# w-k-jones/tobac-flow

Hardware: AMD Instinct MI355X
Metric: Mpix/s end-to-end flow+sobel+watershed, 5424^2 frames (higher is better)
Workload: dtype f32

## Files before the change

tobac_flow_amd/csrc/watershed.hip:

```cpp
#include "tf_common.h"
#include <string.h>
#include <time.h>
#include <stdio.h>
#include <stdlib.h>
#include "tf_prim.h"
#include <new>

typedef unsigned long long u64;
#define WS_INF 0xFFFFFFFFFFFFFFFFull
#define WS_MARKER_BIT 0x8000000000000000ull
#define WS_MAX_NBR 26
#define WS_MAX_DEPTH TF_WS_MAX_DEPTH
#define WS_BATCH 32
#define WS_K2(c, i) ((c).KM[2 * (int64_t)(i)])
#define WS_M1(c, i) ((c).KM[2 * (int64_t)(i) + 1])

struct WsGeom {
    int64_t T; int H, W; int64_t plane;
    int n_nbr;
    int8_t dt[WS_MAX_NBR], dy[WS_MAX_NBR], dx[WS_MAX_NBR];
    int n_tx;
};

#ifndef WS_TILE
#define WS_TILE 16
#endif
__device__ __forceinline__ int64_t ws_vpos(const WsGeom &g, int64_t t, int y, int x) {
    const int64_t tile = (int64_t)(y / WS_TILE) * g.n_tx + x / WS_TILE;
    return ((tile * g.T + t) * WS_TILE + (y % WS_TILE)) * WS_TILE + (x % WS_TILE);
}
static int64_t ws_virtual_voxels(int64_t T, int64_t H, int64_t W) {
    return T * ((H + WS_TILE - 1) / WS_TILE * WS_TILE) * ((W + WS_TILE - 1) / WS_TILE * WS_TILE);
}

struct WsC {
    int64_t R; int n_nbr;
    const u64 *pix; const unsigned *val; const int *nbr;
    u64 *KM;
    u64 *C[WS_MAX_DEPTH], *Rt;
    int *Llo, *Lhi;
    const u64 *emask;
};

__device__ __forceinline__ unsigned ws_ordkey(float v) {
    v = v + 0.0f;
    unsigned u = __float_as_uint(v);
    return (u & 0x80000000u) ? ~u : (u | 0x80000000u);
}
__device__ __forceinline__ u64 ws_load(const u64 *p) {
    return __hip_atomic_load(p, __ATOMIC_RELAXED, __HIP_MEMORY_SCOPE_AGENT);
}
__device__ __forceinline__ int ws_round_flow(float f) {
    return (f == f) ? __float2int_rn(f) : 0;
}

__device__ __forceinline__ int64_t ws_neighbour(const WsGeom &g, int64_t t, int y, int x, int fx, int fy, int bx, int by, int i) {
    const int dt = g.dt[i];
    int yy = y + g.dy[i], xx = x + g.dx[i];
    if (dt == 1) { xx += fx; yy += fy; }
    else if (dt == -1) { xx += bx; yy += by; }
    const int64_t tt = t + dt;
    if (tt < 0 || tt >= g.T || (unsigned)yy >= (unsigned)g.H || (unsigned)xx >= (unsigned)g.W) return -1;
    return tt * g.plane + (int64_t)yy * g.W + xx;
}

__global__ void __launch_bounds__(256)
k_ws_classify(const int32_t *__restrict__ markers, const int8_t *__restrict__ mask, int64_t n, uint8_t *__restrict__ cls)
{
    const int64_t i = (int64_t)blockIdx.x * blockDim.x + threadIdx.x;
    if (i >= n) return;
    const int32_t m = markers[i];
// ... 144 lines not shown
    for (int j = 0; j < 4; j++) { f[j] = ((w >> (8 * j)) & 0xffu) != 0; m[j] = __ballot(f[j]); before += __popcll(m[j] & below); }
    if (y >= g.H || x0 >= g.W) return;
    const int64_t p0 = t * g.plane + (int64_t)y * g.W + x0;
    const int id0 = (int)base[b] + before;
    int c[4], run = 0;
#pragma unroll
    for (int j = 0; j < 4; j++) {
        c[j] = -1;
        if (f[j]) { const int id = id0 + run; c[j] = cls[p0 + j] == 1 ? id : -2 - id; run++; }
    }
    if (x0 + 3 < g.W && (((uintptr_t)(cid + p0)) & 15) == 0) *(int4 *)(cid + p0) = make_int4(c[0], c[1], c[2], c[3]);
    else {
#pragma unroll
        for (int j = 0; j < 4; j++) if (x0 + j < g.W) cid[p0 + j] = c[j];
    }
}
static_assert(WS_TILE * WS_TILE == 256, "one scan block = one tile of one frame");

__global__ void __launch_bounds__(256)
k_ws_cid(const uint8_t *__restrict__ cls, const uint8_t *__restrict__ flag, const int *__restrict__ scan, int64_t n,
         int *__restrict__ cid)
{
    const int64_t i = (int64_t)blockIdx.x * blockDim.x + threadIdx.x;
    if (i >= n) return;
    int c = -1;
    if (flag[i]) c = cls[i] == 1 ? scan[i] : -2 - scan[i];
    cid[i] = c;
}

template <int NN>
__global__ void __launch_bounds__(256)
k_ws_compact(const float *__restrict__ field, const float *__restrict__ fwd, const float *__restrict__ bwd,
             const int *__restrict__ cid, WsGeom g, u64 *__restrict__ pix, unsigned *__restrict__ val,
             int *__restrict__ nbr, u64 *__restrict__ KM, int *__restrict__ nan_flag)
{
    const int x = blockIdx.x * 64 + threadIdx.x, y = blockIdx.y * 4 + threadIdx.y;
    const int64_t t = blockIdx.z;
    if (x >= g.W || y >= g.H) return;
    const int64_t p = t * g.plane + (int64_t)y * g.W + x;
    const int c = cid[p];
    if (c == -1) return;
    const bool marker = c < 0;
    const int64_t id = marker ? -2 - c : c;
    const float2 fw = ((const float2 *)fwd)[p], bw = ((const float2 *)bwd)[p];
    const int fx = ws_round_flow(fw.x), fy = ws_round_flow(fw.y), bx = ws_round_flow(bw.x), by = ws_round_flow(bw.y);
    const float fv = field[p];
    if (fv != fv) *nan_flag = 1;
    const unsigned v = ws_ordkey(fv);
    pix[id] = (u64)p | (marker ? WS_MARKER_BIT : 0ull);
    val[id] = v;
    if (NN > 0) {
        int cn[NN > 0 ? NN : 1];
#pragma unroll
        for (int i = 0; i < NN; i++) {
            const int64_t n = ws_neighbour(g, t, y, x, fx, fy, bx, by, i);
            const int cv = cid[n >= 0 ? n : p];
            cn[i] = n >= 0 ? cv : -1;
        }
#pragma unroll
        for (int i = 0; i < NN; i++) nbr[id * NN + i] = cn[i] < 0 ? -1 : cn[i];
    } else {
        for (int i = 0; i < g.n_nbr; i++) {
            const int64_t n = ws_neighbour(g, t, y, x, fx, fy, bx, by, i);
            int cn = -1;
            if (n >= 0) { cn = cid[n]; if (cn < 0) cn = -1; }
            nbr[id * g.n_nbr + i] = cn;
        }
    }
    *(ulonglong2 *)&KM[2 * id] = make_ulonglong2(marker ? ((u64)v << 32) : WS_INF, WS_INF);
}

struct WsRavel {
    int64_t n; int n_nbr;
    int64_t structure[WS_MAX_NBR]; int32_t floc[WS_MAX_NBR], bloc[WS_MAX_NBR];
    const int32_t *foff, *boff;
};
__device__ __forceinline__ int64_t wsr_neighbour(const WsRavel &g, int64_t p, int fo, int bo, int i) {
    const int64_t n = p + g.structure[i] + (int64_t)g.floc[i] * fo + (int64_t)g.bloc[i] * bo;
    return (n >= 0 && n < g.n) ? n : -1;
}

__global__ void __launch_bounds__(256)
k_wsr_seeds(const int64_t *__restrict__ locs, int64_t n_locs, int64_t n, uint8_t *__restrict__ seed, int *__restrict__ bad)
{
    const int64_t i = (int64_t)blockIdx.x * blockDim.x + threadIdx.x;
    if (i >= n_locs) return;
    const int64_t p = locs[i];
    if (p < 0 || p >= n || (i > 0 && locs[i - 1] >= p)) { *bad = 1; return; }
    seed[p] = 1;
}

__global__ void __launch_bounds__(256)
k_wsr_classify(const uint8_t *__restrict__ seed, const int32_t *__restrict__ output, const int8_t *__restrict__ mask, int64_t n,
               uint8_t *__restrict__ cls, int *__restrict__ bad)
{
    const int64_t i = (int64_t)blockIdx.x * blockDim.x + threadIdx.x;
    if (i >= n) return;
    const bool sd = seed[i] != 0;
    if (sd && output[i] == 0) *bad = 2;
    cls[i] = sd ? 2 : ((mask[i] != 0 && output[i] == 0) ? 1 : 0);
}

__global__ void __launch_bounds__(256)
k_wsr_relevant(const uint8_t *__restrict__ cls, WsRavel g, uint8_t *__restrict__ flag)
{
    const int64_t p = (int64_t)blockIdx.x * blockDim.x + threadIdx.x;
    if (p >= g.n) return;
    const uint8_t c = cls[p];
    uint8_t f = c == 1;
    if (c == 2) {
        const int fo = g.foff[p], bo = g.boff[p];
        for (int i = 0; i < g.n_nbr && !f; i++) { const int64_t n = wsr_neighbour(g, p, fo, bo, i); f |= n >= 0 && cls[n] == 1; }
    }
    flag[p] = f;
}

__global__ void __launch_bounds__(256)
k_wsr_compact(const float *__restrict__ image, const int *__restrict__ cid, WsRavel g, u64 *__restrict__ pix,
              unsigned *__restrict__ val, int *__restrict__ nbr, u64 *__restrict__ KM, int *__restrict__ nan_flag)
{
    const int64_t p = (int64_t)blockIdx.x * blockDim.x + threadIdx.x;
    if (p >= g.n) return;
    const int c = cid[p];
    if (c == -1) return;
    const bool marker = c < 0;
    const int64_t id = marker ? -2 - c : c;
    const int fo = g.foff[p], bo = g.boff[p];
    const float fv = image[p];
    if (fv != fv) *nan_flag = 1;
    const unsigned v = ws_ordkey(fv);
    pix[id] = (u64)p | (marker ? WS_MARKER_BIT : 0ull);
    val[id] = v;
    for (int i = 0; i < g.n_nbr; i++) {
        const int64_t n = wsr_neighbour(g, p, fo, bo, i);
        int cn = -1;
        if (n >= 0) { cn = cid[n]; if (cn < 0) cn = -1; }
        nbr[id * g.n_nbr + i] = cn;
    }
    *(ulonglong2 *)&KM[2 * id] = make_ulonglong2(marker ? ((u64)v << 32) : WS_INF, WS_INF);
}

__global__ void __launch_bounds__(256)
k_wsr_labels(const int *__restrict__ cid, const u64 *__restrict__ Rt, const u64 *__restrict__ pix, int ranked, int32_t *output, int64_t n)
{
    const int64_t i = (int64_t)blockIdx.x * blockDim.x + threadIdx.x;
    if (i >= n) return;
    const int c = cid[i];
    if (c >= 0 && output[i] == 0) { const u64 r = Rt[c]; if (r != WS_INF) output[i] = output[ranked ? (pix[r & 0xFFFFFFFFull] & ~WS_MARKER_BIT) : r]; }
}

__global__ void __launch_bounds__(256)
k_ws_init_level(const u64 *__restrict__ pix, u64 *__restrict__ dst, int64_t R, int is_root, const int *__restrict__ rank)
{
    const int64_t i = (int64_t)blockIdx.x * blockDim.x + threadIdx.x;
    if (i >= R) return;
    const u64 px = pix[i];
    const bool marker = (px & WS_MARKER_BIT) != 0ull;
    const u64 root = rank ? (((u64)(unsigned)rank[i] << 32) | (u64)(unsigned)i) : (px & ~WS_MARKER_BIT);
    dst[i] = marker ? (is_root ? root : 0ull) : WS_INF;
}

__global__ void __launch_bounds__(256)
k_ws_init_labelset(const u64 *__restrict__ pix, const int32_t *__restrict__ markers, int *__restrict__ lo,
                   int *__restrict__ hi, int64_t R)
{
    const int64_t i = (int64_t)blockIdx.x * blockDim.x + threadIdx.x;
    if (i >= R) return;
    const u64 px = pix[i];
    const bool marker = (px & WS_MARKER_BIT) != 0ull;
    const int32_t l = marker ? markers[px & ~WS_MARKER_BIT] : 0;
    lo[i] = marker ? l : 0x7fffffff;
    hi[i] = marker ? l : (int)0x80000000;
}

#define WS_LOCAL_ROUNDS 4
#ifndef WS_LDS_CAP
#define WS_LDS_CAP 4096
#endif
struct WsStage { int cnt[2]; int base; int buf[2][WS_LDS_CAP]; };

__device__ __forceinline__ void ws_stage(WsStage &st, int w, bool enq, int n, int *__restrict__ qout, int *__restrict__ cnt_out, int qcap) {
    if (enq) {
        const int pos = atomicAdd(&st.cnt[w], 1);
        if (pos < WS_LDS_CAP) st.buf[w][pos] = n;
        else { const int g = atomicAdd(cnt_out, 1); if (g < qcap) qout[g] = n; }
    }
}
__device__ __forceinline__ void ws_flush(WsStage &st, int w, int *__restrict__ qout, int *__restrict__ cnt_out, int qcap) {
    __syncthreads();
    const int n = min(st.cnt[w], WS_LDS_CAP);
    if (n > 0) {
        if (threadIdx.x == 0) st.base = atomicAdd(cnt_out, n);
        __syncthreads();
        const int base = st.base;
        for (int i = threadIdx.x; i < n; i += blockDim.x) { const int pos = base + i; if (pos < qcap) qout[pos] = st.buf[w][i]; }
        __syncthreads();
        if (threadIdx.x == 0) st.cnt[w] = 0;
    }
    __syncthreads();
}

template <class Entry>
__device__ __forceinline__ void ws_sweep(int64_t R, const int *__restrict__ qin, const int *__restrict__ cnt_in,
                                         int *__restrict__ qout, int *__restrict__ cnt_out, int qcap, Entry entry)
{
    __shared__ WsStage st;
    if (threadIdx.x == 0) { st.cnt[0] = 0; st.cnt[1] = 0; }
    __syncthreads();
    const int64_t n_in = qin ? (int64_t)min(*cnt_in, qcap) : R;
    const int64_t n_pad = (n_in + 255) & ~255ll;
    for (int64_t i0 = (int64_t)blockIdx.x * 256; i0 < n_pad; i0 += (int64_t)gridDim.x * 256) {
        const int64_t i = i0 + threadIdx.x;
        const bool act = i < n_in;
        int w = 0;
        entry(st, w, act, act ? (qin ? qin[i] : (int)i) : 0);
        for (int r = 0; r < WS_LOCAL_ROUNDS; r++) {
            __syncthreads();
            const int n = min(st.cnt[w], WS_LDS_CAP);
            if (n == 0) break;
            for (int j0 = 0; j0 < n; j0 += 256) {
                const int j = j0 + threadIdx.x;
                const bool a2 = j < n;
                entry(st, w ^ 1, a2, a2 ? st.buf[w][j] : 0);
            }
            __syncthreads();
            if (threadIdx.x == 0) st.cnt[w] = 0;
            w ^= 1;
        }
        ws_flush(st, w, qout, cnt_out, qcap);
    }
}

#define WS_NB 8

template <int NN>
__device__ __forceinline__ void ws_entry_a(const WsC &c, WsStage &st, int w, bool act, int p,
                                           int *__restrict__ qout, int *__restrict__ cnt_out, int qcap)
{
    constexpr int NB = NN ? NN : WS_NB;
    const int n_nbr = NN ? NN : c.n_nbr;
    const int *np = c.nbr + (int64_t)p * n_nbr;
    u64 kp = WS_INF;
    for (int s0 = 0; s0 < n_nbr; s0 += NB) {
        int n[NB];
#pragma unroll
        for (int j = 0; j < NB; j++) n[j] = (act && s0 + j < n_nbr) ? np[s0 + j] : -1;
        if (s0 == 0 && act) kp = ws_load(&WS_K2(c, p));
        const u64 lp = kp >> 32;
        u64 vn[NB], m1[NB], k2[NB];
#pragma unroll
        for (int j = 0; j < NB; j++) {
            const int q = n[j] >= 0 ? n[j] : 0;
            vn[j] = c.val[q];
            const ulonglong2 km = *(const ulonglong2 *)&WS_K2(c, q);
            k2[j] = km.x; m1[j] = km.y;
        }
        u64 cand[NB], old[NB];
#pragma unroll
        for (int j = 0; j < NB; j++) {
            cand[j] = vn[j] > lp ? ((vn[j] << 32) | 1ull) : (vn[j] == lp ? kp + 1ull : kp);
            old[j] = 0ull;
            if (n[j] >= 0) {
                if (kp < m1[j]) atomicMin(&WS_M1(c, n[j]), kp);
                if (cand[j] < k2[j]) old[j] = atomicMin(&WS_K2(c, n[j]), cand[j]);
            }
        }
#pragma unroll
        for (int j = 0; j < NB; j++)
            ws_stage(st, w, n[j] >= 0 && cand[j] < old[j], n[j], qout, cnt_out, qcap);
    }
}

template <int NN>
__global__ void __launch_bounds__(256)
k_ws_sweep_a(WsC c, const int *__restrict__ qin, const int *__restrict__ cnt_in, int *__restrict__ qout,
             int *__restrict__ cnt_out, int qcap)
{
    ws_sweep(c.R, qin, cnt_in, qout, cnt_out, qcap,
             [&](WsStage &st, int w, bool act, int p) { ws_entry_a<NN>(c, st, w, act, p, qout, cnt_out, qcap); });
}

__global__ void __launch_bounds__(256)
k_ws_edge_masks(WsC c, u64 *__restrict__ emask)
{
    const int64_t p = (int64_t)blockIdx.x * blockDim.x + threadIdx.x;
    if (p >= c.R) return;
    const u64 kp = WS_K2(c, p);
    u64 m = 0ull;
    if (kp != WS_INF) {
        const int *np = c.nbr + p * c.n_nbr;
        for (int i0 = 0; i0 < c.n_nbr; i0 += WS_NB) {
            int n[WS_NB]; u64 m1[WS_NB], kn[WS_NB]; unsigned vn[WS_NB];
#pragma unroll
            for (int j = 0; j < WS_NB; j++) n[j] = i0 + j < c.n_nbr ? np[i0 + j] : -1;
#pragma unroll
            for (int j = 0; j < WS_NB; j++) {
                const int q = n[j] >= 0 ? n[j] : 0;
                const ulonglong2 km = *(const ulonglong2 *)&WS_K2(c, q);
                kn[j] = km.x; m1[j] = km.y; vn[j] = c.val[q];
            }
#pragma unroll
            for (int j = 0; j < WS_NB; j++)
                if (n[j] >= 0 && m1[j] == kp) {
                    m |= 1ull << (i0 + j);
                    if ((kn[j] >> 32) == (u64)vn[j] && (kn[j] & 0xFFFFFFFFull) == 1ull) m |= 1ull << (32 + i0 + j);
                }
        }
    }
    emask[p] = m;
}

__device__ __forceinline__ int ws_load_i(const int *p) {
    return __hip_atomic_load(p, __ATOMIC_RELAXED, __HIP_MEMORY_SCOPE_AGENT);
}

template <int NN>
__device__ __forceinline__ void ws_entry_chain(const WsC &c, int k, int depth, u64 *__restrict__ dst, WsStage &st, int w,
                                               bool act0, int p,
                                               int *__restrict__ qout, int *__restrict__ cnt_out, int qcap)
{
    constexpr int NB = NN ? NN : WS_NB;
    const int n_nbr = NN ? NN : c.n_nbr;
    const int *np = c.nbr + (int64_t)p * n_nbr;
    const bool root = k == depth;
    u64 kp = WS_INF, own = WS_INF, em = 0ull;
    int own_lo = 0x7fffffff, own_hi = (int)0x80000000;
    u64 cp[WS_MAX_DEPTH];
    for (int s0 = 0; s0 < n_nbr; s0 += NB) {
        if (s0 == 0 && act0) {
            em = c.emask[p];
            kp = WS_K2(c, p);
            own = ws_load(&dst[p]);
            if (root) { own_lo = ws_load_i(&c.Llo[p]); own_hi = ws_load_i(&c.Lhi[p]); }
            for (int j = 1; j < k; j++) cp[j] = c.C[j][p];
        }
        int n[NB];
#pragma unroll
        for (int j = 0; j < NB; j++) n[j] = (s0 + j < n_nbr && ((em >> (s0 + j)) & 1ull)) ? np[s0 + j] : -1;
        u64 dn[NB];
        int lon[NB], hin[NB];
#pragma unroll
        for (int j = 0; j < NB; j++) {
            dn[j] = WS_INF; lon[j] = 0; hin[j] = 0;
            if (n[j] >= 0) { dn[j] = dst[n[j]]; if (root) { lon[j] = c.Llo[n[j]]; hin[j] = c.Lhi[n[j]]; } }
        }
        u64 offered[NB], old[NB];
        int olo[NB], ohi[NB];
#pragma unroll
        for (int j = 0; j < NB; j++) {
            offered[j] = WS_INF; old[j] = 0ull; olo[j] = (int)0x80000000; ohi[j] = 0x7fffffff;
            if (n[j] >= 0) {
                const bool entry = ((em >> (32 + s0 + j)) & 1ull) != 0ull;
                bool match = true;
                for (int l = 1; l < k && match; l++) {
                    const u64 offered_l = entry ? (l == 1 ? kp : cp[l - 1]) : cp[l];
                    match = offered_l == c.C[l][n[j]];
                }
                if (match) {
                    if (root) offered[j] = own;
                    else offered[j] = entry ? (k == 1 ? kp : cp[k - 1]) : own;
                    if (offered[j] != WS_INF && offered[j] < dn[j]) old[j] = atomicMin(&dst[n[j]], offered[j]);
                    if (root) {
                        if (own_lo < lon[j]) olo[j] = atomicMin(&c.Llo[n[j]], own_lo);
                        if (own_hi > hin[j]) ohi[j] = atomicMax(&c.Lhi[n[j]], own_hi);
                    }
                }
            }
        }
#pragma unroll
        for (int j = 0; j < NB; j++) {
            const bool improved = offered[j] < old[j] || (root && (own_lo < olo[j] || own_hi > ohi[j]));
            ws_stage(st, w, improved, n[j], qout, cnt_out, qcap);
        }
    }
}

template <int NN>
__global__ void __launch_bounds__(256)
k_ws_sweep_chain(WsC c, int k, int depth, const int *__restrict__ qin, const int *__restrict__ cnt_in,
                 int *__restrict__ qout, int *__restrict__ cnt_out, int qcap)
{
    u64 *dst = k == depth ? c.Rt : c.C[k];
    ws_sweep(c.R, qin, cnt_in, qout, cnt_out, qcap,
             [&](WsStage &st, int w, bool act, int p) { ws_entry_chain<NN>(c, k, depth, dst, st, w, act, p, qout, cnt_out, qcap); });
}

__global__ void __launch_bounds__(256)
k_ws_origins(WsC c, int depth, int *__restrict__ org)
{
    const int64_t p = (int64_t)blockIdx.x * blockDim.x + threadIdx.x;
    if (p >= c.R) return;
    const u64 kp = WS_K2(c, p);
    if (kp == WS_INF || c.Rt[p] == WS_INF) return;
    const int lo = c.Llo[p], hi = c.Lhi[p];
    u64 cp[WS_MAX_DEPTH];
    for (int j = 1; j < depth; j++) cp[j] = c.C[j][p];
    const u64 em = c.emask[p];
    for (int i = 0; i < c.n_nbr; i++) {
        if (!((em >> i) & 1ull)) continue;
        const int n = c.nbr[p * c.n_nbr + i];
        const bool entry = ((em >> (32 + i)) & 1ull) != 0ull;
        bool match = true;
        for (int l = 1; l < depth && match; l++) {
            const u64 offered_l = entry ? (l == 1 ? kp : cp[l - 1]) : cp[l];
            match = offered_l == c.C[l][n];
        }
        if (!match) continue;
        if (c.Llo[n] != lo || c.Lhi[n] != hi) {
            const bool complete = depth >= 2 && (c.C[depth - 1][n] & 0xFFFFFFFFull) == 0ull;
            atomicOr(&org[n], complete ? 1 : 2);
        }
    }
}

__global__ void __launch_bounds__(256)
k_ws_count_ambiguous(WsC c, const int *__restrict__ org, unsigned long long *__restrict__ cnt)
{
// ... 315 lines not shown
        TF_CHECK_HIP(tf_exclusive_sum_from(tmp, tb, it, scan + off, (int)carry, (size_t)n, s));
        int last_scan = 0; uint8_t last_flag = 0;
        TF_CHECK_HIP(hipMemcpyAsync(&last_scan, scan + off + n - 1, sizeof(int), hipMemcpyDeviceToHost, s));
        TF_CHECK_HIP(hipMemcpyAsync(&last_flag, flag + off + n - 1, 1, hipMemcpyDeviceToHost, s));
        TF_CHECK_HIP(hipStreamSynchronize(s));
        carry = (int64_t)last_scan + last_flag;
        TF_REQUIRE(carry <= 0x3fffff00ll, "tf_watershed: more than 2^30 relevant pixels in one call (use time windows)");
    }
    *total = carry;
    return TF_OK;
}

static size_t ws_full_bytes(int64_t N, int64_t NV) {
    return tf_align_up((size_t)N, 256) + tf_align_up((size_t)NV, 256) + tf_align_up((size_t)N * 4, 256) + tf_align_up((size_t)NV * 4, 256)
         + tf_align_up(ws_scan_temp_bytes(NV), 256) + tf_align_up((size_t)((N + 255) / 256) * 24 + 64, 256) + 4096;
}
static size_t ws_compact_bytes(int64_t R, int n_nbr, int depth) {
    return tf_align_up((size_t)R * 8, 256) + tf_align_up((size_t)R * 4, 256) + tf_align_up((size_t)R * 4 * n_nbr, 256)
         + (size_t)(depth + 2) * tf_align_up((size_t)R * 8, 256)
         + 2 * tf_align_up((size_t)R * 8 + 256, 256)
         + 5 * tf_align_up((size_t)R * 4, 256) + tf_align_up((size_t)R * 8, 256) + 4096;
}

extern "C" size_t tf_watershed_workspace_bytes(int64_t T, int64_t H, int64_t W, int n_nbr, int chain_depth, int64_t max_relevant)
{
    if (T <= 0 || H <= 0 || W <= 0 || chain_depth < 1 || chain_depth > WS_MAX_DEPTH || n_nbr < 1 || n_nbr > WS_MAX_NBR) return 0;
    const int64_t N = T * H * W;
    if (max_relevant <= 0 || max_relevant > N) max_relevant = N;
    return ws_full_bytes(N, ws_virtual_voxels(T, H, W)) + ws_compact_bytes(max_relevant, n_nbr, chain_depth);
}

struct WsQueues { int *q[2]; int *cnt; int qcap; int *h_cnt; int64_t *processed; };

static int ws_run_phase(const WsC &c, int phase_k, int depth, const WsQueues &Q, hipStream_t s, int64_t max_sweeps,
                        int64_t *sweeps_out, double alg_bytes = 0.0)
{
    const unsigned nbR = (unsigned)((c.R + 255) / 256);
    const unsigned nb = nbR < 2048u ? nbR : 2048u;
    TF_CHECK_HIP(hipMemsetAsync(Q.cnt, 0, (WS_BATCH + 1) * sizeof(int), s));
    int64_t sweeps = 0;
    int parity = 0;
    bool first = true;
    unsigned grid_hint = nb;
    for (;;) {
        const bool scan_batch = first;
        {
            TfProfScope ps(TFK_WS_RELAX, alg_bytes, s);
            alg_bytes = 0.0;
            for (int b = 0; b < WS_BATCH; b++) {
                const int *qin = first ? nullptr : Q.q[parity];
                const unsigned blocks = first ? nbR : grid_hint;
                if (phase_k == 0) {
                    if (c.n_nbr == 6) hipLaunchKernelGGL(k_ws_sweep_a<6>, dim3(blocks), dim3(256), 0, s, c, qin, Q.cnt + b, Q.q[parity ^ 1], Q.cnt + b + 1, Q.qcap);
                    else hipLaunchKernelGGL(k_ws_sweep_a<0>, dim3(blocks), dim3(256), 0, s, c, qin, Q.cnt + b, Q.q[parity ^ 1], Q.cnt + b + 1, Q.qcap);
                } else {
                    if (c.n_nbr == 6) hipLaunchKernelGGL(k_ws_sweep_chain<6>, dim3(blocks), dim3(256), 0, s, c, phase_k, depth, qin, Q.cnt + b, Q.q[parity ^ 1], Q.cnt + b + 1, Q.qcap);
                    else hipLaunchKernelGGL(k_ws_sweep_chain<0>, dim3(blocks), dim3(256), 0, s, c, phase_k, depth, qin, Q.cnt + b, Q.q[parity ^ 1], Q.cnt + b + 1, Q.qcap);
                }
                parity ^= 1;
                first = false;
            }
        }
        TF_CHECK_LAUNCH();
        TF_CHECK_HIP(hipMemcpyAsync(Q.h_cnt, Q.cnt, (WS_BATCH + 1) * sizeof(int), hipMemcpyDeviceToHost, s));
        TF_CHECK_HIP(hipStreamSynchronize(s));
        bool done = false, overflow = false;
        for (int b = (scan_batch ? 1 : 0); b <= WS_BATCH; b++) overflow = overflow || Q.h_cnt[b] > Q.qcap;
        for (int b = (scan_batch ? 1 : 0); b <= WS_BATCH && !overflow; b++) {
            if (Q.h_cnt[b] == 0) { done = true; break; }
            if (b < WS_BATCH) *Q.processed += Q.h_cnt[b];
        }
        sweeps += WS_BATCH;
        {
            const int64_t last = Q.h_cnt[WS_BATCH];
            int64_t gb = (last * 4 + 255) / 256;
            if (gb < 64) gb = 64;
            if (gb > (int64_t)nb) gb = nb;
            grid_hint = (unsigned)gb;
        }
        if (done) break;
        if (sweeps > max_sweeps) { tf_set_error("tf_watershed: phase %d did not converge in %lld sweeps", phase_k, (long long)sweeps); return TF_ENOCONV; }
        if (overflow) {
            first = true;
            TF_CHECK_HIP(hipMemsetAsync(Q.cnt, 0, (WS_BATCH + 1) * sizeof(int), s));
            continue;
        }
        TF_CHECK_HIP(hipMemcpyAsync(Q.cnt, Q.cnt + WS_BATCH, sizeof(int), hipMemcpyDeviceToDevice, s));
        TF_CHECK_HIP(hipMemsetAsync(Q.cnt + 1, 0, WS_BATCH * sizeof(int), s));
    }
    *sweeps_out = sweeps;
// ... 328 lines not shown
    hipStream_t s = j->s;
    const WsC &c = j->c;
    const int64_t R = j->R;
    const unsigned nbr_blocks = (unsigned)((R + 255) / 256);
    hipLaunchKernelGGL(k_ws_init_level, dim3(nbr_blocks), dim3(256), 0, s, c.pix, c.Rt, R, 1, ranked ? (const int *)j->rank_dev : (const int *)nullptr);
    hipLaunchKernelGGL(k_ws_init_labelset, dim3(nbr_blocks), dim3(256), 0, s, c.pix, j->markers, c.Llo, c.Lhi, R);
    TF_CHECK_LAUNCH();
    int64_t sw = 0;
    const int rc = ws_run_phase(c, j->depth, j->depth, j->Q, s, j->max_sweeps, &sw);
    if (rc) return rc;
    if (j->speculate_fast && j->depth == 1) j->st[1] = sw; else j->st[2 + (j->depth < 3 ? j->depth - 1 : 2)] += sw;
    j->st[12] += 1;
    TF_CHECK_HIP(hipMemsetAsync(j->org, 0, (size_t)R * sizeof(int), s));
    TF_CHECK_HIP(hipMemsetAsync(j->d_cnt, 0, 4 * sizeof(unsigned long long), s));
    hipLaunchKernelGGL(k_ws_origins, dim3(nbr_blocks), dim3(256), 0, s, c, j->depth, j->org);
    hipLaunchKernelGGL(k_ws_count_ambiguous, dim3(nbr_blocks), dim3(256), 0, s, c, j->org, j->d_cnt);
    TF_CHECK_LAUNCH();
    TF_CHECK_HIP(hipMemcpyAsync(j->h_amb, j->d_cnt, 4 * sizeof(unsigned long long), hipMemcpyDeviceToHost, s));
    TF_CHECK_HIP(hipStreamSynchronize(s));
    return TF_OK;
}

static int ws_job_sweeps(tf_ws_job *j)
{
    if (!j->sweeps_pending) return TF_OK;
    j->sweeps_pending = false;
    int64_t *st = j->st;
    const WsC &c = j->c;
    hipStream_t s = j->s;
    const unsigned nbr_blocks = (unsigned)((j->R + 255) / 256);
    int rc = ws_run_phase(c, 0, j->depth_max, j->Q, s, j->max_sweeps, &st[0], 29.0 * (double)j->N);
    if (rc) return rc;
    {
        TfProfScope ps(TFK_WS_SETUP, 0.0, s);
        hipLaunchKernelGGL(k_ws_edge_masks, dim3(nbr_blocks), dim3(256), 0, s, c, (u64 *)c.emask);
    }
    TF_CHECK_LAUNCH();
    j->speculate_fast = !((j->flags & TF_WS_SKIP_FAST_PATH) && j->depth0 > 1);
    st[5] = j->speculate_fast ? 0 : -1;
    j->depth = j->depth0;
    j->root_pending = true;
    if (j->speculate_fast) {
        j->depth = 1;
        rc = ws_root_and_check(j, false);
        if (rc) return rc;
        st[5] = j->h_amb[2] != 0;
        if (j->h_amb[2] == 0 || j->depth_max <= 1) j->root_pending = false;
        else j->depth = j->depth0;
    }
    if (j->root_pending) {
        rc = ws_chain_levels(j);
        if (rc) return rc;
    }
    st[8] = j->depth; st[9] = (int64_t)j->h_amb[0]; st[10] = (int64_t)j->h_amb[1]; st[11] = (int64_t)j->h_amb[2];
    return TF_OK;
}

static int ws_job_begin(tf_ws_job *j, const float *field, const int32_t *markers, const int8_t *mask,
                        const float *fwd, const float *bwd, int64_t T, int64_t H, int64_t W,
                        const int8_t *nbr_host, int n_nbr, int depth0, int depth_max, int flags,
                        void *ws, size_t ws_bytes, void *stream,
                        const WsRavel *rv = nullptr, const int64_t *rv_locs = nullptr, int64_t rv_n_locs = 0, int64_t spec_key = -1)
{
    int64_t *st = j->st;
    for (int i = 0; i < TF_WS_NSTATS; i++) st[i] = 0;
    TF_REQUIRE((flags & ~(TF_WS_SKIP_FAST_PATH | TF_WS_REFERENCE_ORDER | TF_WS_DEFER_SWEEPS)) == 0, "tf_watershed: unknown flag");
// ... 74 lines not shown
            long long *t_count = (long long *)scan, *t_base = t_count + n_tiles;
            hipLaunchKernelGGL(k_ws_count_tiles, dim3((unsigned)((n_tiles + 3) / 4)), dim3(256), 0, s, (const uint8_t *)flag, n_tiles, t_count);
            size_t tb = scan_bytes;
            TF_CHECK_HIP(tf_exclusive_sum(scan_tmp, tb, (const long long *)t_count, t_base, (size_t)n_tiles, s));
            long long h_last[2] = {0, 0};
            TF_CHECK_HIP(hipMemcpyAsync(&h_last[0], t_base + n_tiles - 1, sizeof(long long), hipMemcpyDeviceToHost, s));
            TF_CHECK_HIP(hipMemcpyAsync(&h_last[1], t_count + n_tiles - 1, sizeof(long long), hipMemcpyDeviceToHost, s));
            TF_CHECK_HIP(hipStreamSynchronize(s));
            R = h_last[0] + h_last[1];
            TF_REQUIRE(R <= 0x3fffff00ll, "tf_watershed: more than 2^30 relevant pixels in one call (use time windows)");
        } else {
            const int rc_scan = ws_scan_flags(flag, scan, NV, scan_tmp, scan_bytes, s, &R);
            if (rc_scan) return rc_scan;
        }
    }
    st[6] = R;
    j->R = R;
    if (ws_bytes < ws_full_bytes(N, NV) + ws_compact_bytes(R > 0 ? R : 1, n_nbr, depth_max)) {
        tf_set_error("tf_watershed: workspace too small for %lld relevant pixels", (long long)R);
        return TF_ENOMEM;
    }
    if (rv) hipLaunchKernelGGL(k_ws_cid, dim3(nb1), dim3(256), 0, s, cls, flag, scan, N, cid);
    else if (tiles) hipLaunchKernelGGL(k_ws_cid_tiles, dim3((unsigned)((NV / 256 + 3) / 4)), dim3(256), 0, s, (const uint8_t *)cls, (const uint8_t *)flag,
                                       (const long long *)((long long *)scan + NV / 256), NV / 256, g, cid);
    else hipLaunchKernelGGL(k_ws_cid_tiled, grid, block, 0, s, (const uint8_t *)cls, (const uint8_t *)flag, (const int *)scan, g, cid);
    TF_CHECK_LAUNCH();
    WsC &c = j->c; memset(&c, 0, sizeof(c));
    c.R = R; c.n_nbr = n_nbr;
    j->org = nullptr; j->rank_dev = nullptr;
    j->depth = 0;
    if (R > 0) {
        u64 *pix = ar.take<u64>(R); unsigned *val = ar.take<unsigned>(R); int *nbr = ar.take<int>(R * n_nbr);
        c.pix = pix; c.val = val; c.nbr = nbr;
        c.KM = ar.take<u64>(2 * R);
        for (int k = 1; k < depth_max; k++) c.C[k] = ar.take<u64>(R);
        c.Rt = ar.take<u64>(R);
        c.Llo = ar.take<int>(R); c.Lhi = ar.take<int>(R); j->org = ar.take<int>(R);
        j->rank_dev = ar.take<int>(R);
        u64 *emask = ar.take<u64>(R);
        c.emask = emask;
        WsQueues &Q = j->Q;
        Q.qcap = (int)(2 * R < 0x7fffff00ll ? 2 * R : 0x7fffff00ll);
        Q.q[0] = ar.take<int>(2 * R + 64); Q.q[1] = ar.take<int>(2 * R + 64);
        j->subid = ar.take<int>(R);
        Q.cnt = d_flags; Q.h_cnt = j->h_cnt; Q.processed = &st[7];
        if (!ar.ok()) { tf_set_error("tf_watershed: workspace too small"); return TF_ENOMEM; }
        int *d_nan = d_flags + WS_BATCH + 4;
        TF_CHECK_HIP(hipMemsetAsync(d_nan, 0, sizeof(int), s));
        {
            TfProfScope ps(TFK_WS_SETUP, 0.0, s);
            if (rv) hipLaunchKernelGGL(k_wsr_compact, dim3(nb1), dim3(256), 0, s, field, (const int *)cid, *rv, pix, val, nbr, c.KM, d_nan);
            else if (n_nbr == 6) hipLaunchKernelGGL(k_ws_compact<6>, grid, block, 0, s, field, fwd, bwd, cid, g, pix, val, nbr, c.KM, d_nan);
            else if (n_nbr == 18) hipLaunchKernelGGL(k_ws_compact<18>, grid, block, 0, s, field, fwd, bwd, cid, g, pix, val, nbr, c.KM, d_nan);
            else if (n_nbr == 26) hipLaunchKernelGGL(k_ws_compact<26>, grid, block, 0, s, field, fwd, bwd, cid, g, pix, val, nbr, c.KM, d_nan);
            else hipLaunchKernelGGL(k_ws_compact<0>, grid, block, 0, s, field, fwd, bwd, cid, g, pix, val, nbr, c.KM, d_nan);
        }
        TF_CHECK_LAUNCH();
        {
            int h_nan = 0;
            TF_CHECK_HIP(hipMemcpyAsync(&h_nan, d_nan, sizeof(int), hipMemcpyDeviceToHost, s));
            TF_CHECK_HIP(hipStreamSynchronize(s));
            if (h_nan) {
                tf_set_error("tf_watershed: the field is NaN at a floodable pixel or at a seed next to one; the pop order of the "
                             "reference's heap is undefined for NaN keys (detection.get_combined_edge_field maps NaN to +inf)");
                return TF_EINVAL;
            }
        }
        const int64_t max_sweeps = rv ? 4096 + 2 * R : 4096 + 512 * (T + H + W);
        j->max_sweeps = max_sweeps;
        if ((flags & TF_WS_REFERENCE_ORDER) && spec_key >= 0) {
            j->vmax = (unsigned)spec_key;
            j->speculative = true;
            const int rc_x = ws_job_export(j);
            if (rc_x) return rc_x;
        }
        j->sweeps_pending = true;
        if (flags & TF_WS_DEFER_SWEEPS) return TF_OK;
        return ws_job_sweeps(j);
    }
    st[8] = j->depth; st[9] = (int64_t)j->h_amb[0]; st[10] = (int64_t)j->h_amb[1]; st[11] = (int64_t)j->h_amb[2];
    return TF_OK;
}

static int ws_job_replay(tf_ws_job *j)
{
    if (!j->need_replay || j->replay_done) return j->replay_rc;
    const double t0 = ws_now_ms();
    int n_ranked = 0;
// ... 318 lines not shown
```

Measured before the change: 1026.

## Split K2/M1 arrays, defer M1 relaxation, specialise chain sweeps by depth

Replaces the interleaved K2/M1 array with two separate arrays. M1 updates move out of the iterative phase-0 sweep into one pass run after convergence. The chain sweep kernels get templates on level K and on root/non-root, so loops unroll, per-thread arrays shrink, and the root-only Llo/Lhi loads are skipped elsewhere. 6-neighbour kernels are capped at 64 VGPRs and the LDS staging capacity is halved, both to raise occupancy. The risks are register spills under the VGPR cap, more staging overflow into global queues with the smaller LDS buffer, and one extra full pass for M1.

```diff
diff --git a/tobac_flow_amd/csrc/watershed.hip b/tobac_flow_amd/csrc/watershed.hip
--- a/tobac_flow_amd/csrc/watershed.hip
+++ b/tobac_flow_amd/csrc/watershed.hip
@@ -12,8 +12,8 @@
 #define WS_MAX_NBR 26
 #define WS_MAX_DEPTH TF_WS_MAX_DEPTH
 #define WS_BATCH 32
-#define WS_K2(c, i) ((c).KM[2 * (int64_t)(i)])
-#define WS_M1(c, i) ((c).KM[2 * (int64_t)(i) + 1])
+#define WS_K2(c, i) ((c).K2[(int64_t)(i)])
+#define WS_M1(c, i) ((c).M1[(int64_t)(i)])
 
 struct WsGeom {
     int64_t T; int H, W; int64_t plane;
@@ -36,7 +36,7 @@
 struct WsC {
     int64_t R; int n_nbr;
     const u64 *pix; const unsigned *val; const int *nbr;
-    u64 *KM;
+    u64 *K2, *M1;
     u64 *C[WS_MAX_DEPTH], *Rt;
     int *Llo, *Lhi;
     const u64 *emask;
@@ -247,7 +247,7 @@
 __global__ void __launch_bounds__(256)
 k_ws_compact(const float *__restrict__ field, const float *__restrict__ fwd, const float *__restrict__ bwd,
              const int *__restrict__ cid, WsGeom g, u64 *__restrict__ pix, unsigned *__restrict__ val,
-             int *__restrict__ nbr, u64 *__restrict__ KM, int *__restrict__ nan_flag)
+             int *__restrict__ nbr, u64 *__restrict__ K2, u64 *__restrict__ M1, int *__restrict__ nan_flag)
 {
     const int x = blockIdx.x * 64 + threadIdx.x, y = blockIdx.y * 4 + threadIdx.y;
     const int64_t t = blockIdx.z;
@@ -282,7 +282,8 @@
             nbr[id * g.n_nbr + i] = cn;
         }
     }
-    *(ulonglong2 *)&KM[2 * id] = make_ulonglong2(marker ? ((u64)v << 32) : WS_INF, WS_INF);
+    K2[id] = marker ? ((u64)v << 32) : WS_INF;
+    M1[id] = WS_INF;
 }
 
 struct WsRavel {
@@ -332,7 +333,7 @@
 
 __global__ void __launch_bounds__(256)
 k_wsr_compact(const float *__restrict__ image, const int *__restrict__ cid, WsRavel g, u64 *__restrict__ pix,
-              unsigned *__restrict__ val, int *__restrict__ nbr, u64 *__restrict__ KM, int *__restrict__ nan_flag)
+              unsigned *__restrict__ val, int *__restrict__ nbr, u64 *__restrict__ K2, u64 *__restrict__ M1, int *__restrict__ nan_flag)
 {
     const int64_t p = (int64_t)blockIdx.x * blockDim.x + threadIdx.x;
     if (p >= g.n) return;
@@ -352,7 +353,8 @@
         if (n >= 0) { cn = cid[n]; if (cn < 0) cn = -1; }
         nbr[id * g.n_nbr + i] = cn;
     }
-    *(ulonglong2 *)&KM[2 * id] = make_ulonglong2(marker ? ((u64)v << 32) : WS_INF, WS_INF);
+    K2[id] = marker ? ((u64)v << 32) : WS_INF;
+    M1[id] = WS_INF;
 }
 
 __global__ void __launch_bounds__(256)
@@ -390,7 +392,7 @@
 
 #define WS_LOCAL_ROUNDS 4
 #ifndef WS_LDS_CAP
-#define WS_LDS_CAP 4096
+#define WS_LDS_CAP 2048
 #endif
 struct WsStage { int cnt[2]; int base; int buf[2][WS_LDS_CAP]; };
 
@@ -448,6 +450,10 @@
 
 #define WS_NB 8
 
+__device__ __forceinline__ u64 ws_cand_a(unsigned vn, unsigned lp, u64 kp) {
+    return vn > lp ? (((u64)vn << 32) | 1ull) : (vn == lp ? kp + 1ull : kp);
+}
+
 template <int NN>
 __device__ __forceinline__ void ws_entry_a(const WsC &c, WsStage &st, int w, bool act, int p,
                                            int *__restrict__ qout, int *__restrict__ cnt_out, int qcap)
@@ -461,38 +467,65 @@
 #pragma unroll
         for (int j = 0; j < NB; j++) n[j] = (act && s0 + j < n_nbr) ? np[s0 + j] : -1;
         if (s0 == 0 && act) kp = ws_load(&WS_K2(c, p));
-        const u64 lp = kp >> 32;
-        u64 vn[NB], m1[NB], k2[NB];
+        const unsigned lp = (unsigned)(kp >> 32);
+        unsigned vn[NB];
+        u64 k2[NB];
 #pragma unroll
         for (int j = 0; j < NB; j++) {
             const int q = n[j] >= 0 ? n[j] : 0;
             vn[j] = c.val[q];
-            const ulonglong2 km = *(const ulonglong2 *)&WS_K2(c, q);
-            k2[j] = km.x; m1[j] = km.y;
-        }
-        u64 cand[NB], old[NB];
+            k2[j] = WS_K2(c, q);
+        }
 #pragma unroll
         for (int j = 0; j < NB; j++) {
-            cand[j] = vn[j] > lp ? ((vn[j] << 32) | 1ull) : (vn[j] == lp ? kp + 1ull : kp);
-            old[j] = 0ull;
-            if (n[j] >= 0) {
-                if (kp < m1[j]) atomicMin(&WS_M1(c, n[j]), kp);
-                if (cand[j] < k2[j]) old[j] = atomicMin(&WS_K2(c, n[j]), cand[j]);
-            }
+            const u64 cand = ws_cand_a(vn[j], lp, kp);
+            const bool go = n[j] >= 0 && cand < k2[j];
+            k2[j] = 0ull;
+            if (go) k2[j] = atomicMin(&WS_K2(c, n[j]), cand);
         }
 #pragma unroll
         for (int j = 0; j < NB; j++)
-            ws_stage(st, w, n[j] >= 0 && cand[j] < old[j], n[j], qout, cnt_out, qcap);
-    }
-}
-
-template <int NN>
+            ws_stage(st, w, n[j] >= 0 && ws_cand_a(vn[j], lp, kp) < k2[j], n[j], qout, cnt_out, qcap);
+    }
+}
+
 __global__ void __launch_bounds__(256)
 k_ws_sweep_a(WsC c, const int *__restrict__ qin, const int *__restrict__ cnt_in, int *__restrict__ qout,
              int *__restrict__ cnt_out, int qcap)
 {
     ws_sweep(c.R, qin, cnt_in, qout, cnt_out, qcap,
-             [&](WsStage &st, int w, bool act, int p) { ws_entry_a<NN>(c, st, w, act, p, qout, cnt_out, qcap); });
+             [&](WsStage &st, int w, bool act, int p) { ws_entry_a<0>(c, st, w, act, p, qout, cnt_out, qcap); });
+}
+__global__ void __launch_bounds__(256) __attribute__((amdgpu_num_vgpr(64)))
+k_ws_sweep_a6(WsC c, const int *__restrict__ qin, const int *__restrict__ cnt_in, int *__restrict__ qout,
+              int *__restrict__ cnt_out, int qcap)
+{
+    ws_sweep(c.R, qin, cnt_in, qout, cnt_out, qcap,
+             [&](WsStage &st, int w, bool act, int p) { ws_entry_a<6>(c, st, w, act, p, qout, cnt_out, qcap); });
+}
+
+template <int NN>
+__global__ void __launch_bounds__(256)
+k_ws_sweep_m1(WsC c)
+{
+    const int64_t p = (int64_t)blockIdx.x * blockDim.x + threadIdx.x;
+    if (p >= c.R) return;
+    const u64 kp = WS_K2(c, p);
+    if (kp == WS_INF) return;
+    constexpr int NB = NN ? NN : WS_NB;
+    const int n_nbr = NN ? NN : c.n_nbr;
+    const int *np = c.nbr + p * n_nbr;
+    for (int s0 = 0; s0 < n_nbr; s0 += NB) {
+        int n[NB];
+        u64 m1[NB];
+#pragma unroll
+        for (int j = 0; j < NB; j++) n[j] = s0 + j < n_nbr ? np[s0 + j] : -1;
+#pragma unroll
+        for (int j = 0; j < NB; j++) m1[j] = WS_M1(c, n[j] >= 0 ? n[j] : 0);
+#pragma unroll
+        for (int j = 0; j < NB; j++)
+            if (n[j] >= 0 && kp < m1[j]) atomicMin(&WS_M1(c, n[j]), kp);
+    }
 }
 
 __global__ void __launch_bounds__(256)
@@ -511,8 +544,7 @@
 #pragma unroll
             for (int j = 0; j < WS_NB; j++) {
                 const int q = n[j] >= 0 ? n[j] : 0;
-                const ulonglong2 km = *(const ulonglong2 *)&WS_K2(c, q);
-                kn[j] = km.x; m1[j] = km.y; vn[j] = c.val[q];
+                kn[j] = WS_K2(c, q); m1[j] = WS_M1(c, q); vn[j] = c.val[q];
             }
 #pragma unroll
             for (int j = 0; j < WS_NB; j++)
@@ -529,75 +561,103 @@
     return __hip_atomic_load(p, __ATOMIC_RELAXED, __HIP_MEMORY_SCOPE_AGENT);
 }
 
-template <int NN>
-__device__ __forceinline__ void ws_entry_chain(const WsC &c, int k, int depth, u64 *__restrict__ dst, WsStage &st, int w,
+template <int NN, int K, bool ROOT>
+__device__ __forceinline__ void ws_entry_chain(const WsC &c, int k_rt, u64 *__restrict__ dst, const u64 *__restrict__ below, WsStage &st, int w,
                                                bool act0, int p,
                                                int *__restrict__ qout, int *__restrict__ cnt_out, int qcap)
 {
     constexpr int NB = NN ? NN : WS_NB;
     const int n_nbr = NN ? NN : c.n_nbr;
+    const int k = K ? K : k_rt;
     const int *np = c.nbr + (int64_t)p * n_nbr;
-    const bool root = k == depth;
     u64 kp = WS_INF, own = WS_INF, em = 0ull;
     int own_lo = 0x7fffffff, own_hi = (int)0x80000000;
-    u64 cp[WS_MAX_DEPTH];
+    u64 cp[K ? K : 1];
+    u64 ek = WS_INF;
+    auto offer = [&](int i, int l) -> u64 {
+        const bool entry = ((em >> (32 + i)) & 1ull) != 0ull;
+        if constexpr (K != 0) return entry ? (l == 1 ? kp : cp[l - 1]) : cp[l];
+        else return entry ? (l == 1 ? kp : c.C[l - 1][p]) : c.C[l][p];
+    };
+    auto offer_k = [&](int i) -> u64 {
+        const bool entry = ((em >> (32 + i)) & 1ull) != 0ull;
+        return (ROOT || !entry) ? own : ek;
+    };
     for (int s0 = 0; s0 < n_nbr; s0 += NB) {
         if (s0 == 0 && act0) {
             em = c.emask[p];
             kp = WS_K2(c, p);
             own = ws_load(&dst[p]);
-            if (root) { own_lo = ws_load_i(&c.Llo[p]); own_hi = ws_load_i(&c.Lhi[p]); }
-            for (int j = 1; j < k; j++) cp[j] = c.C[j][p];
+            if constexpr (ROOT) { own_lo = ws_load_i(&c.Llo[p]); own_hi = ws_load_i(&c.Lhi[p]); }
+            if constexpr (K != 0) {
+#pragma unroll
+                for (int j = 1; j < K; j++) cp[j] = c.C[j][p];
+            }
+            if constexpr (!ROOT) {
+                if constexpr (K == 1) ek = kp;
+                else if constexpr (K != 0) ek = cp[K - 1];
+                else ek = k == 1 ? kp : below[p];
+            }
         }
         int n[NB];
 #pragma unroll
         for (int j = 0; j < NB; j++) n[j] = (s0 + j < n_nbr && ((em >> (s0 + j)) & 1ull)) ? np[s0 + j] : -1;
         u64 dn[NB];
-        int lon[NB], hin[NB];
+        int lon[ROOT ? NB : 1], hin[ROOT ? NB : 1];
 #pragma unroll
         for (int j = 0; j < NB; j++) {
-            dn[j] = WS_INF; lon[j] = 0; hin[j] = 0;
-            if (n[j] >= 0) { dn[j] = dst[n[j]]; if (root) { lon[j] = c.Llo[n[j]]; hin[j] = c.Lhi[n[j]]; } }
-        }
-        u64 offered[NB], old[NB];
-        int olo[NB], ohi[NB];
+            dn[j] = WS_INF;
+            if constexpr (ROOT) { lon[j] = 0; hin[j] = 0; }
+            if (n[j] >= 0) { dn[j] = dst[n[j]]; if constexpr (ROOT) { lon[j] = c.Llo[n[j]]; hin[j] = c.Lhi[n[j]]; } }
+        }
 #pragma unroll
         for (int j = 0; j < NB; j++) {
-            offered[j] = WS_INF; old[j] = 0ull; olo[j] = (int)0x80000000; ohi[j] = 0x7fffffff;
+            const u64 seen = dn[j];
+            dn[j] = 0ull;
+            int seen_lo = 0, seen_hi = 0;
+            if constexpr (ROOT) { seen_lo = lon[j]; seen_hi = hin[j]; lon[j] = (int)0x80000000; hin[j] = 0x7fffffff; }
             if (n[j] >= 0) {
-                const bool entry = ((em >> (32 + s0 + j)) & 1ull) != 0ull;
                 bool match = true;
-                for (int l = 1; l < k && match; l++) {
-                    const u64 offered_l = entry ? (l == 1 ? kp : cp[l - 1]) : cp[l];
-                    match = offered_l == c.C[l][n[j]];
+                if constexpr (K != 0) {
+#pragma unroll
+                    for (int l = 1; l < K; l++) if (match) match = offer(s0 + j, l) == c.C[l][n[j]];
+                } else {
+                    for (int l = 1; l < k && match; l++) match = offer(s0 + j, l) == c.C[l][n[j]];
                 }
                 if (match) {
-                    if (root) offered[j] = own;
-                    else offered[j] = entry ? (k == 1 ? kp : cp[k - 1]) : own;
-                    if (offered[j] != WS_INF && offered[j] < dn[j]) old[j] = atomicMin(&dst[n[j]], offered[j]);
-                    if (root) {
-                        if (own_lo < lon[j]) olo[j] = atomicMin(&c.Llo[n[j]], own_lo);
-                        if (own_hi > hin[j]) ohi[j] = atomicMax(&c.Lhi[n[j]], own_hi);
+                    const u64 offered = offer_k(s0 + j);
+                    if (offered != WS_INF && offered < seen) dn[j] = atomicMin(&dst[n[j]], offered);
+                    if constexpr (ROOT) {
+                        if (own_lo < seen_lo) lon[j] = atomicMin(&c.Llo[n[j]], own_lo);
+                        if (own_hi > seen_hi) hin[j] = atomicMax(&c.Lhi[n[j]], own_hi);
                     }
                 }
             }
         }
 #pragma unroll
         for (int j = 0; j < NB; j++) {
-            const bool improved = offered[j] < old[j] || (root && (own_lo < olo[j] || own_hi > ohi[j]));
+            bool improved = offer_k(s0 + j) < dn[j];
+            if constexpr (ROOT) improved = improved || own_lo < lon[j] || own_hi > hin[j];
             ws_stage(st, w, improved, n[j], qout, cnt_out, qcap);
         }
     }
 }
 
-template <int NN>
-__global__ void __launch_bounds__(256)
-k_ws_sweep_chain(WsC c, int k, int depth, const int *__restrict__ qin, const int *__restrict__ cnt_in,
+template <bool ROOT>
+__global__ void __launch_bounds__(256)
+k_ws_sweep_chain(WsC c, int k, u64 *__restrict__ dst, const u64 *__restrict__ below, const int *__restrict__ qin, const int *__restrict__ cnt_in,
                  int *__restrict__ qout, int *__restrict__ cnt_out, int qcap)
 {
-    u64 *dst = k == depth ? c.Rt : c.C[k];
     ws_sweep(c.R, qin, cnt_in, qout, cnt_out, qcap,
-             [&](WsStage &st, int w, bool act, int p) { ws_entry_chain<NN>(c, k, depth, dst, st, w, act, p, qout, cnt_out, qcap); });
+             [&](WsStage &st, int w, bool act, int p) { ws_entry_chain<0, 0, ROOT>(c, k, dst, below, st, w, act, p, qout, cnt_out, qcap); });
+}
+template <int K, bool ROOT>
+__global__ void __launch_bounds__(256) __attribute__((amdgpu_num_vgpr(64)))
+k_ws_sweep_chain6(WsC c, int k, u64 *__restrict__ dst, const u64 *__restrict__ below, const int *__restrict__ qin, const int *__restrict__ cnt_in,
+                  int *__restrict__ qout, int *__restrict__ cnt_out, int qcap)
+{
+    ws_sweep(c.R, qin, cnt_in, qout, cnt_out, qcap,
+             [&](WsStage &st, int w, bool act, int p) { ws_entry_chain<6, K, ROOT>(c, k, dst, below, st, w, act, p, qout, cnt_out, qcap); });
 }
 
 __global__ void __launch_bounds__(256)
@@ -979,6 +1039,22 @@
 
 struct WsQueues { int *q[2]; int *cnt; int qcap; int *h_cnt; int64_t *processed; };
 
+template <int NN, bool ROOT>
+static void ws_launch_chain(unsigned blocks, hipStream_t s, const WsC &c, int k, const int *qin, const int *cnt_in,
+                            int *qout, int *cnt_out, int qcap)
+{
+    u64 *dst = ROOT ? c.Rt : c.C[k];
+    const u64 *below = (!ROOT && k > 1) ? c.C[k - 1] : nullptr;
+    if constexpr (NN == 6) {
+        if (k == 1) hipLaunchKernelGGL((k_ws_sweep_chain6<1, ROOT>), dim3(blocks), dim3(256), 0, s, c, k, dst, below, qin, cnt_in, qout, cnt_out, qcap);
+        else if (k == 2) hipLaunchKernelGGL((k_ws_sweep_chain6<2, ROOT>), dim3(blocks), dim3(256), 0, s, c, k, dst, below, qin, cnt_in, qout, cnt_out, qcap);
+        else if (k == 3) hipLaunchKernelGGL((k_ws_sweep_chain6<3, ROOT>), dim3(blocks), dim3(256), 0, s, c, k, dst, below, qin, cnt_in, qout, cnt_out, qcap);
+        else hipLaunchKernelGGL((k_ws_sweep_chain6<0, ROOT>), dim3(blocks), dim3(256), 0, s, c, k, dst, below, qin, cnt_in, qout, cnt_out, qcap);
+    } else {
+        hipLaunchKernelGGL((k_ws_sweep_chain<ROOT>), dim3(blocks), dim3(256), 0, s, c, k, dst, below, qin, cnt_in, qout, cnt_out, qcap);
+    }
+}
+
 static int ws_run_phase(const WsC &c, int phase_k, int depth, const WsQueues &Q, hipStream_t s, int64_t max_sweeps,
                         int64_t *sweeps_out, double alg_bytes = 0.0)
 {
@@ -997,12 +1073,16 @@
             for (int b = 0; b < WS_BATCH; b++) {
                 const int *qin = first ? nullptr : Q.q[parity];
                 const unsigned blocks = first ? nbR : grid_hint;
+                int *qout = Q.q[parity ^ 1];
                 if (phase_k == 0) {
-                    if (c.n_nbr == 6) hipLaunchKernelGGL(k_ws_sweep_a<6>, dim3(blocks), dim3(256), 0, s, c, qin, Q.cnt + b, Q.q[parity ^ 1], Q.cnt + b + 1, Q.qcap);
-                    else hipLaunchKernelGGL(k_ws_sweep_a<0>, dim3(blocks), dim3(256), 0, s, c, qin, Q.cnt + b, Q.q[parity ^ 1], Q.cnt + b + 1, Q.qcap);
+                    if (c.n_nbr == 6) hipLaunchKernelGGL(k_ws_sweep_a6, dim3(blocks), dim3(256), 0, s, c, qin, Q.cnt + b, qout, Q.cnt + b + 1, Q.qcap);
+                    else hipLaunchKernelGGL(k_ws_sweep_a, dim3(blocks), dim3(256), 0, s, c, qin, Q.cnt + b, qout, Q.cnt + b + 1, Q.qcap);
+                } else if (phase_k == depth) {
+                    if (c.n_nbr == 6) ws_launch_chain<6, true>(blocks, s, c, phase_k, qin, Q.cnt + b, qout, Q.cnt + b + 1, Q.qcap);
+                    else ws_launch_chain<0, true>(blocks, s, c, phase_k, qin, Q.cnt + b, qout, Q.cnt + b + 1, Q.qcap);
                 } else {
-                    if (c.n_nbr == 6) hipLaunchKernelGGL(k_ws_sweep_chain<6>, dim3(blocks), dim3(256), 0, s, c, phase_k, depth, qin, Q.cnt + b, Q.q[parity ^ 1], Q.cnt + b + 1, Q.qcap);
-                    else hipLaunchKernelGGL(k_ws_sweep_chain<0>, dim3(blocks), dim3(256), 0, s, c, phase_k, depth, qin, Q.cnt + b, Q.q[parity ^ 1], Q.cnt + b + 1, Q.qcap);
+                    if (c.n_nbr == 6) ws_launch_chain<6, false>(blocks, s, c, phase_k, qin, Q.cnt + b, qout, Q.cnt + b + 1, Q.qcap);
+                    else ws_launch_chain<0, false>(blocks, s, c, phase_k, qin, Q.cnt + b, qout, Q.cnt + b + 1, Q.qcap);
                 }
                 parity ^= 1;
                 first = false;
@@ -1397,6 +1477,11 @@
     int rc = ws_run_phase(c, 0, j->depth_max, j->Q, s, j->max_sweeps, &st[0], 29.0 * (double)j->N);
     if (rc) return rc;
     {
+        TfProfScope ps(TFK_WS_RELAX, 0.0, s);
+        if (c.n_nbr == 6) hipLaunchKernelGGL(k_ws_sweep_m1<6>, dim3(nbr_blocks), dim3(256), 0, s, c);
+        else hipLaunchKernelGGL(k_ws_sweep_m1<0>, dim3(nbr_blocks), dim3(256), 0, s, c);
+    }
+    {
         TfProfScope ps(TFK_WS_SETUP, 0.0, s);
         hipLaunchKernelGGL(k_ws_edge_masks, dim3(nbr_blocks), dim3(256), 0, s, c, (u64 *)c.emask);
     }
@@ -1537,7 +1622,7 @@
     if (R > 0) {
         u64 *pix = ar.take<u64>(R); unsigned *val = ar.take<unsigned>(R); int *nbr = ar.take<int>(R * n_nbr);
         c.pix = pix; c.val = val; c.nbr = nbr;
-        c.KM = ar.take<u64>(2 * R);
+        c.K2 = ar.take<u64>(R); c.M1 = ar.take<u64>(R);
         for (int k = 1; k < depth_max; k++) c.C[k] = ar.take<u64>(R);
         c.Rt = ar.take<u64>(R);
         c.Llo = ar.take<int>(R); c.Lhi = ar.take<int>(R); j->org = ar.take<int>(R);
@@ -1554,11 +1639,11 @@
         TF_CHECK_HIP(hipMemsetAsync(d_nan, 0, sizeof(int), s));
         {
             TfProfScope ps(TFK_WS_SETUP, 0.0, s);
-            if (rv) hipLaunchKernelGGL(k_wsr_compact, dim3(nb1), dim3(256), 0, s, field, (const int *)cid, *rv, pix, val, nbr, c.KM, d_nan);
-            else if (n_nbr == 6) hipLaunchKernelGGL(k_ws_compact<6>, grid, block, 0, s, field, fwd, bwd, cid, g, pix, val, nbr, c.KM, d_nan);
-            else if (n_nbr == 18) hipLaunchKernelGGL(k_ws_compact<18>, grid, block, 0, s, field, fwd, bwd, cid, g, pix, val, nbr, c.KM, d_nan);
-            else if (n_nbr == 26) hipLaunchKernelGGL(k_ws_compact<26>, grid, block, 0, s, field, fwd, bwd, cid, g, pix, val, nbr, c.KM, d_nan);
-            else hipLaunchKernelGGL(k_ws_compact<0>, grid, block, 0, s, field, fwd, bwd, cid, g, pix, val, nbr, c.KM, d_nan);
+            if (rv) hipLaunchKernelGGL(k_wsr_compact, dim3(nb1), dim3(256), 0, s, field, (const int *)cid, *rv, pix, val, nbr, c.K2, c.M1, d_nan);
+            else if (n_nbr == 6) hipLaunchKernelGGL(k_ws_compact<6>, grid, block, 0, s, field, fwd, bwd, cid, g, pix, val, nbr, c.K2, c.M1, d_nan);
+            else if (n_nbr == 18) hipLaunchKernelGGL(k_ws_compact<18>, grid, block, 0, s, field, fwd, bwd, cid, g, pix, val, nbr, c.K2, c.M1, d_nan);
+            else if (n_nbr == 26) hipLaunchKernelGGL(k_ws_compact<26>, grid, block, 0, s, field, fwd, bwd, cid, g, pix, val, nbr, c.K2, c.M1, d_nan);
+            else hipLaunchKernelGGL(k_ws_compact<0>, grid, block, 0, s, field, fwd, bwd, cid, g, pix, val, nbr, c.K2, c.M1, d_nan);
         }
         TF_CHECK_LAUNCH();
         {
```

Result: faster. 1054 (median of 6 runs) (+2.7%).
